# tyb311/TCCT

Hardware: AMD Instinct MI355X
Metric: OCT B-scans/sec fwd+bwd(+clip+AdamW), stc_tt bs=8 1x800x1100 (higher is better)
Workload: dtype bf16; 1 GPU; stc_tt --los=di bs=8/GPU 1x800x1100 (net tensors 3x800x1104); global_batch=8, parallelism=dp1, ranks=1, grad_allreduce=none, slowest_step=88

## Files before the change

### include/tcct_hip.h

```cpp
#ifndef TCCT_HIP_H
#define TCCT_HIP_H
#include <stdint.h>
#ifdef __cplusplus
extern "C" {
#endif

typedef void* tcct_stream_t;

enum { TCCT_F32 = 0, TCCT_BF16 = 1 };
enum { TCCT_ACT_NONE = 0, TCCT_ACT_LRELU = 1, TCCT_ACT_HSWISH = 2, TCCT_ACT_GELU = 3, TCCT_ACT_SIGMOID = 4,
       TCCT_ACT_ABS = 5 };
enum { TCCT_CRIT_DICE = 0, TCCT_CRIT_DICE2 = 1, TCCT_CRIT_IOU = 2, TCCT_CRIT_MSE = 3 };
enum { TCCT_MCRIT_DICE = 0, TCCT_MCRIT_DICE2 = 1, TCCT_MCRIT_IOU = 2, TCCT_MCRIT_CE = 3 };

int tcct_version(void);
const char* tcct_last_error(void);
int tcct_set_outputs_prezeroed(int on);

int tcct_image_to_nhwc4(const float* img, void* out, int N, int Csrc, int H, int Wsrc, int Wdst, int dtype,
                        tcct_stream_t stream);
int tcct_u8_gather2d(const uint8_t* src, uint8_t* dst, int N, int SH, int SW, int C, int sy0, int sx0, int sh, int sw, int DH, int DW,
                     int dy0, int dx0, int dh, int dw, int flipy, int flipx, int mul, int div, int fill, tcct_stream_t stream);
int tcct_onehot_to_index(const int64_t* onehot, uint8_t* lab, int N, int C, int64_t HW, tcct_stream_t stream);
int tcct_labels_to_u8(const int64_t* lab, uint8_t* out, int N, int H, int Wsrc, int Wdst, tcct_stream_t stream);
// ... 199 lines not shown
int tcct_c3_wgrad(const void* x4, const void* dy, float* dw, float* dbias, int B, int H, int W, int stride, tcct_stream_t stream);
int tcct_c3_bn_fwd_train(const void* x4, const float* w, const float* bias, void* z, int B, int H, int W, int stride, double* sums,
                         const float* gamma, const float* beta, float eps, float momentum, float* running_mean, float* running_var,
                         int64_t* num_batches_tracked, float* mean_rstd, float* ab, int post_act, tcct_stream_t stream);
int tcct_c3_bn_fwd_eval(const void* x4, const float* w, const float* bias, void* z, int B, int H, int W, int stride, const float* ab, int post_act,
                        tcct_stream_t stream);
int tcct_c3_bn_bwd_reduce(const void* x4, const float* w, const float* bias, const void* dz, int B, int H, int W, int stride, const float* ab,
                          double* raw, int post_act, tcct_stream_t stream);
int tcct_c3_bn_bwd_wgrad(const void* x4, const float* w, const float* bias, const void* dz, int B, int H, int W, int stride, const float* coef,
                         float* dw, float* dbias, int post_act, tcct_stream_t stream);
int64_t tcct_c3_bn_bwd_prefetch(int tiles_ahead);
int tcct_c3_bn_bwd_onepass(const void* x4, const float* w, const float* bias, const void* dz, int B, int H, int W, int stride, const float* mean_rstd,
                           const float* ab, float* work, double* sums, float* dw, float* dbias, float* dgamma, float* dbeta, int post_act, tcct_stream_t stream);
int tcct_pw_wgrad_smalln(const void* x, const void* dy, float* dw, float* dbias, int64_t M, int K, int N, int x_dtype,
                         int dy_dtype, tcct_stream_t stream);

int tcct_stream_copy(const void* src, void* dst, int64_t nbytes, tcct_stream_t stream);

int64_t tcct_kernel_census(int which, int reset);
int tcct_marker(int id, tcct_stream_t stream);

int tcct_dwconv3x3_fwd(const void* x, const float* w, const float* bias, void* y, int N, int H, int W, int C,
                       int stride, int add_input, int dtype, tcct_stream_t stream);
int tcct_dwconv3x3_fwd_bnstats(const void* x, const float* w, const float* bias, void* y, int N, int H, int W, int C, int stride,
                               int add_input, double* stats, int dtype, tcct_stream_t stream);
int tcct_dwconv3x3_dgrad(const void* dy, const float* w, void* dx, int N, int H, int W, int C, int stride,
                         int add_input, int dtype, tcct_stream_t stream);
int tcct_dwconv3x3_dgrad_add(const void* dy, const float* w, const void* res, void* dx, int N, int H, int W, int C, int stride,
                             int add_input, int dtype, tcct_stream_t stream);
int tcct_dwconv3x3_wgrad(const void* x, const void* dy, float* dw, float* dbias, int N, int H, int W, int C,
                         int stride, int dtype, tcct_stream_t stream);
int tcct_dwconv3x3_fwd_xaff(const void* x, const float* xab, const float* w, const float* bias, void* y, int N, int H, int W, int C, int stride,
                            double* stats, int dtype, tcct_stream_t stream);
int tcct_dwconv3x3_wgrad_xaff(const void* x, const float* xab, const void* dy, float* dw, float* dbias, int N, int H, int W, int C, int stride, int dtype,
                              tcct_stream_t stream);
int tcct_dwconv3x3_dgrad_bnred(const void* dy, const float* w, const void* y_prev, const float* ab_prev, void* dx, double* raw, int N, int H, int W, int C,
                               int dtype, tcct_stream_t stream);

int tcct_metapool_fwd(const void* x, void* y, int B, int64_t N, int C, int dtype, tcct_stream_t stream);
int tcct_metapool_bwd(const void* dy, void* dx, int B, int64_t N, int C, int dtype, tcct_stream_t stream);
int tcct_metapool_residual_fwd(const void* x, const void* res, const float* scale, void* y, int B, int64_t N, int C, int dtype,
                               tcct_stream_t stream);
int tcct_metapool_scaled_bwd(const void* dy, const float* scale, void* dx, int B, int64_t N, int C, int dtype, tcct_stream_t stream);
int tcct_ln_metapool_residual_fwd(const void* t, void* y, int B, int64_t N, int C, const float* gamma, const float* beta, float eps, const float* scale,
                                  int dtype, tcct_stream_t stream);
int tcct_ln_metapool_residual_ln_fwd(const void* t, void* y, void* y2, int B, int64_t N, int C, const float* gamma, const float* beta, float eps,
                                     const float* scale, const float* gamma2, const float* beta2, float eps2, float* mean_rstd2, int dtype, tcct_stream_t stream);
int tcct_ln_metapool_residual_bwd(const void* t, const void* dy, void* dt, int B, int64_t N, int C, const float* gamma, float eps, const float* scale,
                                  float* dgamma, float* dbeta, int dtype, tcct_stream_t stream);
int tcct_maxpool2_fwd(const void* x, void* y, int N, int H, int W, int C, int dtype, tcct_stream_t stream);
int tcct_maxpool2_bwd(const void* x, const void* dy, void* dx, int N, int H, int W, int C, int dtype, tcct_stream_t stream);
int tcct_maxpool2_bwd_add(const void* x, const void* dy, const void* res, void* dx, int N, int H, int W, int C, int dtype,
                          tcct_stream_t stream);
int tcct_bilinear_fwd(const void* x, void* y, int N, int H, int W, int C, int Ho, int Wo, int align_corners, int dtype,
                      tcct_stream_t stream);
int tcct_bilinear_bwd_separable(const float* dy, float* dx, float* workspace, int N, int H, int W, int C, int Ho, int Wo,
                                int align_corners, tcct_stream_t stream);
int tcct_bilinear_add_fwd(const void* x, const void* res, void* y, int N, int H, int W, int C, int Ho, int Wo, int align_corners,
                          int dtype, tcct_stream_t stream);
int64_t tcct_bilinear_bwd_x2(int on);
int tcct_bilinear_bwd(const void* dy, void* dx, int N, int H, int W, int C, int Ho, int Wo, int align_corners, int dtype,
                      tcct_stream_t stream);
int tcct_l2norm_fwd(const void* x, void* y, int64_t M, int C, float eps, int dtype, tcct_stream_t stream);
int tcct_l2norm_bwd(const void* x, const void* dy, void* dx, int64_t M, int C, float eps, int dtype, tcct_stream_t stream);
int tcct_l2norm_bwd_scaled(const void* x, const void* dy, void* dx, int64_t M, int C, float eps, float scale, int dtype,
                           tcct_stream_t stream);
int tcct_l2norm_bwd_scaled_add(const void* x, const void* dy, const void* res, void* dx, int64_t M, int C, float eps, float scale, int dtype,
                               tcct_stream_t stream);
int tcct_normadd_fwd(const void* g0, const void* g1, const void* g2, float* inv1, float* inv2, void* out, int N, int H, int W, int C,
                     int h1, int w1, int h2, int w2, float eps, int dtype, tcct_stream_t stream);
int tcct_normadd6_fwd(const void* a0, const void* b0, const void* a1, const void* b1, const void* a2, const void* b2, float* inv1, float* inv2,
                      void* out, int N, int H, int W, int C, int h1, int w1, int h2, int w2, float eps, int dtype, tcct_stream_t stream);
int tcct_l2norm_bwd2_scaled(const void* xa, const void* xb, const void* dn, const void* res_a, const void* res_b, void* da, void* db,
                            int64_t M, int C, float eps, float scale, int dtype, tcct_stream_t stream);

int tcct_softmax_dice_fwd(const void* logits, const uint8_t* labels, int64_t M, int C, double* sums, float* loss,
                          int dtype, tcct_stream_t stream);
int tcct_softmax_dice_bwd(const void* logits, const uint8_t* labels, int64_t M, int C, const double* sums,
                          const float* grad_out, float grad_scale, void* dlogits, int dtype, tcct_stream_t stream);
int tcct_updice_fwd(const float* low, const uint8_t* labels, int B, int h, int w, int H, int W, int C, double* sums, float* loss,
                    tcct_stream_t stream);
int tcct_updice_bwd(const float* low, const uint8_t* labels, int B, int h, int w, int H, int W, int C, const double* sums,
                    const float* grad_out, float grad_scale, float* ws, float* dlow, tcct_stream_t stream);
int tcct_dice_ds_fwd(const void* logits, int dtype, const uint8_t* labels, int B, int H, int W, int C, const float* low1, int h1, int w1, const float* low2,
                     int h2, int w2, const float* low3, int h3, int w3, float coff, double* sums, float* loss, tcct_stream_t stream);
int tcct_softmax_crit_fwd(const void* logits, const uint8_t* labels, int64_t M, int C, int kind, const float* class_w, double* sums, float* loss, int dtype,
                          tcct_stream_t stream);
int tcct_softmax_crit_bwd(const void* logits, const uint8_t* labels, int64_t M, int C, int kind, const float* class_w, const double* sums, const float* grad_out,
                          float grad_scale, void* dlogits, int dtype, tcct_stream_t stream);
int tcct_upcrit_fwd(const float* low, const uint8_t* labels, int B, int h, int w, int H, int W, int C, int kind, const float* class_w, double* sums, float* loss,
                    tcct_stream_t stream);
int tcct_upcrit_bwd(const float* low, const uint8_t* labels, int B, int h, int w, int H, int W, int C, int kind, const float* class_w, const double* sums,
                    const float* grad_out, float grad_scale, float* ws, float* dlow, tcct_stream_t stream);
int tcct_crit_ds_fwd(const void* logits, int dtype, const uint8_t* labels, int B, int H, int W, int C, const float* low1, int h1, int w1, const float* low2, int h2, int w2,
                     const float* low3, int h3, int w3, float coff, int kind, const float* class_w, double* sums, float* loss, tcct_stream_t stream);
int tcct_softmax_mcrit_fwd(const void* logits, const uint8_t* labels, int B, int64_t HW, int C, int kind, const float* class_w, double* sums, float* loss, int dtype,
                           tcct_stream_t stream);
int tcct_softmax_mcrit_bwd(const void* logits, const uint8_t* labels, int B, int64_t HW, int C, int kind, const float* class_w, const double* sums, const float* grad_out,
                           float grad_scale, void* dlogits, int dtype, tcct_stream_t stream);
int tcct_upmcrit_fwd(const float* low, const uint8_t* labels, int B, int h, int w, int H, int W, int C, int kind, const float* class_w, double* sums, float* loss,
                     tcct_stream_t stream);
int tcct_upmcrit_bwd(const float* low, const uint8_t* labels, int B, int h, int w, int H, int W, int C, int kind, const float* class_w, const double* sums,
                     const float* grad_out, float grad_scale, float* ws, float* dlow, tcct_stream_t stream);
int tcct_mcrit_ds_fwd(const void* logits, int dtype, const uint8_t* labels, int B, int H, int W, int C, const float* low1, int h1, int w1, const float* low2, int h2, int w2,
                      const float* low3, int h3, int w3, float coff, int kind, const float* class_w, double* sums, float* loss, tcct_stream_t stream);
int tcct_softmax_pick(const void* logits, const uint8_t* labels, int64_t M, int C, float* prob_lab, uint8_t* argmax,
                      int dtype, tcct_stream_t stream);
int tcct_confusion_counts(const uint8_t* pred, const uint8_t* labels, int N, int64_t HW, int C, float* out,
                          tcct_stream_t stream);

int tcct_gate_fusion_fwd(const void* x1, const void* x2, const float* field, void* y, int N, int H, int W, int C, int hs, int ws,
                         int dtype, tcct_stream_t stream);
int tcct_gate_fusion_bwd(const void* dy, const float* field, void* dx1, void* dx2, int N, int H, int W, int C, int hs, int ws,
                         int dtype, tcct_stream_t stream);

int tcct_mask_boundaries(const uint8_t* mask, int32_t* out, int N, int H, int W, int C, tcct_stream_t stream);

int tcct_eval_counts(const void* pred, int pred_kind, const uint8_t* labels, int B, int H, int W, int C, int h_valid, int w_valid, int32_t* counts, int32_t* bnd_pred,
                     int32_t* bnd_lab, uint8_t* argmax, tcct_stream_t stream);
int tcct_eval_scores(const int32_t* counts, const int32_t* bnd_pred, const int32_t* bnd_lab, int B, int C, int W, int h_valid, int w_valid, double* table,
                     tcct_stream_t stream);
int tcct_ordered_decode(const void* logits, int kind, int B, int H, int W, int C, int h_valid, int w_valid, void* take_ws, uint8_t* mask, int32_t* bnd,
                        int32_t* changed, int32_t* best, tcct_stream_t stream);
int64_t tcct_layout_decode_ws_bytes(int B, int H, int W, int S, int n_free);
int tcct_layout_decode(const void* pred, int kind, int B, int H, int W, int C, const int* layers, int S, int free_mask, int h_valid, int w_valid, void* ws,
                       uint8_t* mask, int32_t* bnd, int32_t* changed, int32_t* best, uint8_t* state, tcct_stream_t stream);
int tcct_eval_layout_scores(const int32_t* counts, const int32_t* bnd_pred, const int32_t* bnd_lab, int B, int C, int S, int W, int h_valid, int w_valid,
                            double* table, tcct_stream_t stream);
int64_t tcct_layout_marginals_ws_bytes(int B, int H, int W, int S, int n_free);
int tcct_layout_marginals(const void* logits, int kind, int B, int H, int W, int C, const int* layers, int S, int free_mask, int h_valid, int w_valid, float tau,
                          void* ws, float* surf, float* var, float* logz, float* post, tcct_stream_t stream);
int tcct_eval_soft_scores(const float* surf, const float* var, const int32_t* bnd_lab, int B, int S, int W, int h_valid, int w_valid, double* table,
                          tcct_stream_t stream);

int tcct_slice_channels_fwd(const void* x, float* y, int64_t M, int C, int start, int n, int dtype, tcct_stream_t stream);
int tcct_slice_channels_bwd(const float* dy, void* dx, int64_t M, int C, int start, int n, int dtype, tcct_stream_t stream);
int tcct_label_planes(const uint8_t* labels, float* onehot, float* edge, int N, int H, int W, int start, int n,
                      tcct_stream_t stream);
int tcct_gumbel_colsoftmax_fwd(const float* x, const float* eps, float* out, float* stats, int N, int H, int W, int CH,
                               tcct_stream_t stream);
int tcct_gumbel_colsoftmax_bwd(const float* x, const float* eps, const float* stats, const float* dout, float* dx, int N,
                               int H, int W, int CH, tcct_stream_t stream);
int tcct_colsoftmax_fwd(const float* x, float* y, int N, int H, int W, tcct_stream_t stream);
int tcct_colsoftmax_bwd(const float* y, const float* dy, float* dx, int N, int H, int W, tcct_stream_t stream);
int tcct_colwsum_fwd(const float* x, const float* wts, float* out, int N, int H, int W, tcct_stream_t stream);
int tcct_colwsum_bwd(const float* dout, const float* wts, float* dx, int N, int H, int W, tcct_stream_t stream);
int tcct_mse_fwd(const float* a, const float* b, int64_t n, double* acc, float* out, tcct_stream_t stream);
int tcct_mse_bwd(const float* a, const float* b, int64_t n, const float* grad_out, float grad_scale, float* da, float* db,
                 tcct_stream_t stream);

int64_t tcct_fpl_select_workspace_bytes();
int tcct_fpl_select(const void* feat, const uint8_t* labels, const float* prob, int64_t M, int C, void* workspace, uint32_t* counts,
                    uint8_t* binmap, float* pro_sum, int dtype, tcct_stream_t stream);
int tcct_fpl_loss(const float* pro_sum, const uint32_t* counts, const float* buf_grad, int C, float* pro, float* loss, float* dpro_over_n,
                  tcct_stream_t stream);
int tcct_fpl_backward(const uint8_t* labels, const uint8_t* binmap, const float* dpro_over_n, const float* grad_out,
                      float grad_scale, int64_t M, void* dfeat, int dtype, tcct_stream_t stream);
int tcct_l2norm_bwd_fplgrad(const void* x, const uint8_t* labels, const uint8_t* binmap, const float* dpro_over_n, const float* grad_out,
                            float grad_scale, int ncls, const void* res, void* dx, int64_t M, float eps, float scale, int dtype, tcct_stream_t stream);
int tcct_bilinear_bwd_fplgrad(const uint8_t* labels, const uint8_t* binmap, const float* dpro_over_n, const float* grad_out, float grad_scale, int ncls,
                              void* dx, int N, int H, int W, int Ho, int Wo, int align_corners, int dtype, tcct_stream_t stream);
int tcct_l2norm_bwd2_fplgrad(const void* xa, const void* xb, const uint8_t* labels, const uint8_t* binmap, const float* dpro_over_n,
                             const float* grad_out, float grad_scale, int ncls, const void* res_a, const void* res_b, void* da, void* db,
                             int64_t M, float eps, float scale, int dtype, tcct_stream_t stream);

int64_t tcct_fatt_kstats_workspace_bytes(int B, int64_t N, int C);
// ... 42 lines not shown
```

### tcct_amd/csrc/loss.hip

```cpp
#include "common.h"

#define LB 256
#define MAXC 5
#define MCNS mc5
#include "loss_classes.inc"
#undef MCNS
#undef MAXC
#define MAXC 8

#define MCNS mc8
#include "loss_classes.inc"
#undef MCNS
#undef MAXC
#define MAXC 16
#define MCNS mc16
#include "loss_classes.inc"
#undef MCNS

#define DICE_BY_C(CALL) (C == 5 ? mc5::CALL : (C <= 8 ? mc8::CALL : mc16::CALL))
#define PICK_BY_C(CALL) (C <= 8 ? mc8::CALL : mc16::CALL)

extern "C" int tcct_softmax_dice_fwd(const void* logits, const uint8_t* labels, int64_t M, int C, double* sums, float* loss, int dtype, tcct_stream_t stream) {
    return DICE_BY_C(tcct_softmax_dice_fwd_impl(logits, labels, M, C, sums, loss, dtype, stream));
}
extern "C" int tcct_softmax_dice_bwd(const void* logits, const uint8_t* labels, int64_t M, int C, const double* sums, const float* grad_out, float grad_scale, void* dlogits, int dtype, tcct_stream_t stream) {
    return DICE_BY_C(tcct_softmax_dice_bwd_impl(logits, labels, M, C, sums, grad_out, grad_scale, dlogits, dtype, stream));
}
extern "C" int tcct_updice_fwd(const float* low, const uint8_t* labels, int B, int h, int w, int H, int W, int C, double* sums, float* loss, tcct_stream_t stream) {
    return DICE_BY_C(tcct_updice_fwd_impl(low, labels, B, h, w, H, W, C, sums, loss, stream));
}
extern "C" int tcct_updice_bwd(const float* low, const uint8_t* labels, int B, int h, int w, int H, int W, int C, const double* sums, const float* grad_out, float grad_scale, float* ws, float* dlow, tcct_stream_t stream) {
    return DICE_BY_C(tcct_updice_bwd_impl(low, labels, B, h, w, H, W, C, sums, grad_out, grad_scale, ws, dlow, stream));
}
extern "C" int tcct_dice_ds_fwd(const void* logits, int dtype, const uint8_t* labels, int B, int H, int W, int C, const float* low1, int h1, int w1,
                                const float* low2, int h2, int w2, const float* low3, int h3, int w3, float coff, double* sums, float* loss,
                                tcct_stream_t stream) {
    const float* lows[3] = {low1, low2, low3};
    const int lh[3] = {h1, h2, h3}, lw[3] = {w1, w2, w3};
    const int nlow = low1 ? (low2 ? (low3 ? 3 : 2) : 1) : 0;
    return DICE_BY_C(tcct_dice_ds_fwd_impl(logits, dtype, labels, B, H, W, C, lows, lh, lw, nlow, coff, sums, loss, stream));
}
extern "C" int tcct_softmax_pick(const void* logits, const uint8_t* labels, int64_t M, int C, float* prob_lab, uint8_t* argmax, int dtype, tcct_stream_t stream) {
    return PICK_BY_C(tcct_softmax_pick_impl(logits, labels, M, C, prob_lab, argmax, dtype, stream));
}
extern "C" int tcct_confusion_counts(const uint8_t* pred, const uint8_t* labels, int N, int64_t HW, int C, float* out, tcct_stream_t stream) {
    return PICK_BY_C(tcct_confusion_counts_impl(pred, labels, N, HW, C, out, stream));
}

template <typename T>
__global__ void k_slice_fwd(const T* __restrict__ x, float* __restrict__ y, int64_t M, int C, int start, int n) {
    for (int64_t i = (int64_t)blockIdx.x * blockDim.x + threadIdx.x; i < M * n; i += (int64_t)gridDim.x * blockDim.x)
        y[i] = ldf(x + (i / n) * C + start + (i % n));
}
template <typename T>
__global__ void k_slice_bwd(const float* __restrict__ dy, T* __restrict__ dx, int64_t M, int C, int start, int n) {
    for (int64_t i = (int64_t)blockIdx.x * blockDim.x + threadIdx.x; i < M * C; i += (int64_t)gridDim.x * blockDim.x) {
        int c = (int)(i % C) - start;
        stf(dx + i, (c >= 0 && c < n) ? dy[(i / C) * n + c] : 0.f);
    }
}
extern "C" int tcct_slice_channels_fwd(const void* x, float* y, int64_t M, int C, int start, int n, int dtype, tcct_stream_t stream) {
    TCCT_CHECK(start >= 0 && n > 0 && start + n <= C, "slice_channels_fwd: bad range");
    TCCT_DISPATCH(dtype, hipLaunchKernelGGL(k_slice_fwd<T>, dim3(tcct_grid(M * n, LB, 1 << 16)), dim3(LB), 0, (hipStream_t)stream, (const T*)x, y, M, C, start, n));
    TCCT_LAUNCH_OK();
}
extern "C" int tcct_slice_channels_bwd(const float* dy, void* dx, int64_t M, int C, int start, int n, int dtype, tcct_stream_t stream) {
    TCCT_CHECK(start >= 0 && n > 0 && start + n <= C, "slice_channels_bwd: bad range");
    TCCT_DISPATCH(dtype, hipLaunchKernelGGL(k_slice_bwd<T>, dim3(tcct_grid(M * C, LB, 1 << 16)), dim3(LB), 0, (hipStream_t)stream, dy, (T*)dx, M, C, start, n));
    TCCT_LAUNCH_OK();
}

__global__ void k_label_planes(const uint8_t* __restrict__ lab, float* __restrict__ onehot, float* __restrict__ edge, int N,
                               int H, int W, int start, int n) {
    const int64_t total = (int64_t)N * H * W;
    for (int64_t i = (int64_t)blockIdx.x * blockDim.x + threadIdx.x; i < total; i += (int64_t)gridDim.x * blockDim.x) {
        int l = lab[i];
        if (onehot)
            for (int c = 0; c < n; ++c) onehot[i * n + c] = (l == start + c) ? 1.f : 0.f;
        if (edge) {
            int h = (int)((i / W) % H);
            float e = 0.f;
            if (h > 0) {
                int lp = lab[i - W];
                int cnt = 0;
                if (l != lp) { cnt += (l >= start && l < start + n); cnt += (lp >= start && lp < start + n); }
                e = cnt > 0 ? 1.f : 0.f;
            }
            edge[i] = e;
        }
    }
}
extern "C" int tcct_label_planes(const uint8_t* labels, float* onehot, float* edge, int N, int H, int W, int start, int n,
                                 tcct_stream_t stream) {
    hipLaunchKernelGGL(k_label_planes, dim3(tcct_grid((int64_t)N * H * W, LB, 1 << 16)), dim3(LB), 0, (hipStream_t)stream, labels, onehot, edge, N, H, W, start, n);
    TCCT_LAUNCH_OK();
}

#define GSEG 8
__device__ __forceinline__ float gumbel_z(float x, float e) { return x - 0.5f * logf(-logf(e)); }

template <int CH>
__global__ void __launch_bounds__(64 * GSEG)
k_gumbel_fwd(const float* __restrict__ x, const float* __restrict__ eps, float* __restrict__ out,
             float* __restrict__ stats, int N, int H, int W) {
    __shared__ float sm[GSEG][64], sz[GSEG][64];
    const int WC = W * CH;
    const int64_t cols = (int64_t)N * WC;
    const int lane = threadIdx.x & 63, seg = threadIdx.x >> 6;
    const int64_t col = (int64_t)blockIdx.x * 64 + lane;
    const bool ok = col < cols;
    const int64_t cc = ok ? col : 0;
    const int64_t n = cc / WC;
    const int wc = (int)(cc % WC);
    const float* xp = x + n * (int64_t)H * WC + wc;
    const float* ep = eps + n * (int64_t)H * WC + wc;
// ... 281 lines not shown
```

### tcct_amd/csrc/loss_classes.inc

```
namespace MCNS {
#include "loss_device.inc"
__device__ __forceinline__ void dice_accum(float (&z)[MAXC], int C, int l, float (&I)[MAXC], float (&P)[MAXC], float (&G)[MAXC]) {
    softmax_inplace(z, C);
#pragma unroll
    for (int c = 0; c < MAXC; ++c) {
        P[c] += z[c];
        if (c == l) { I[c] += z[c]; G[c] += 1.f; }
    }
}
#define DSB 1024
template <typename T>
__global__ void __launch_bounds__(DSB) k_dice_sums(const T* __restrict__ logits, const uint8_t* __restrict__ lab, int64_t M, int C,
                            double* __restrict__ sums ) {
    float I[MAXC], P[MAXC], G[MAXC];
#pragma unroll
    for (int c = 0; c < MAXC; ++c) I[c] = P[c] = G[c] = 0.f;
    for (int64_t i = (int64_t)blockIdx.x * blockDim.x + threadIdx.x; i < M; i += (int64_t)gridDim.x * blockDim.x) {
        float z[MAXC];
#pragma unroll
        for (int c = 0; c < MAXC; ++c) z[c] = c < C ? ldf(logits + i * C + c) : -INFINITY;
        dice_accum(z, C, lab[i], I, P, G);
    }
    sums_block_tail<DSB>(I, P, G, C, sums);
}
// ... 18 lines not shown
    __shared__ float s_k[2 * MAXC];
    if ((int)threadIdx.x < C) {
        const int c = threadIdx.x;
        const double U = 1.0 + sums[C + c] + sums[2 * C + c];
        s_k[c] = (float)(-2.0 / U);
        s_k[MAXC + c] = (float)((1.0 + 2.0 * sums[c]) / (U * U));
    }
    __syncthreads();
#pragma unroll
    for (int c = 0; c < MAXC; ++c) { ka[c] = c < C ? s_k[c] : 0.f; kb[c] = c < C ? s_k[MAXC + c] : 0.f; }
}

template <typename T>
__global__ void k_dice_bwd(const T* __restrict__ logits, const uint8_t* __restrict__ lab, int64_t M, int C,
                           const double* __restrict__ sums, const float* __restrict__ gout, float gscale,
                           T* __restrict__ dlogits) {
    float a[MAXC], b[MAXC];
    const float gs = gscale * (gout ? *gout : 1.f);
    dice_grad_coeffs(sums, C, a, b);
    for (int64_t i = (int64_t)blockIdx.x * blockDim.x + threadIdx.x; i < M; i += (int64_t)gridDim.x * blockDim.x) {
        float z[MAXC], mx = -INFINITY;
#pragma unroll
        for (int c = 0; c < MAXC; ++c) { z[c] = c < C ? ldf(logits + i * C + c) : -INFINITY; mx = fmaxf(mx, z[c]); }
        float s = 0.f;
#pragma unroll
        for (int c = 0; c < MAXC; ++c) { z[c] = c < C ? __expf(z[c] - mx) : 0.f; s += z[c]; }
        float inv = __builtin_amdgcn_rcpf(s);
        int l = lab[i];
        float dp[MAXC], dot = 0.f;
#pragma unroll
        for (int c = 0; c < MAXC; ++c) { z[c] *= inv; dp[c] = b[c] + (c == l ? a[c] : 0.f); dot += z[c] * dp[c]; }
#pragma unroll
        for (int c = 0; c < MAXC; ++c)
            if (c < C) stf(dlogits + i * C + c, gs * z[c] * (dp[c] - dot));
    }
}
static int tcct_softmax_dice_bwd_impl(const void* logits, const uint8_t* labels, int64_t M, int C, const double* sums,
                                     const float* grad_out, float grad_scale, void* dlogits, int dtype, tcct_stream_t stream) {
    TCCT_CHECK(C >= 2 && C <= MAXC, "softmax_dice_bwd: C=%d unsupported", C);
    TCCT_DISPATCH(dtype, hipLaunchKernelGGL(k_dice_bwd<T>, dim3(tcct_grid(M, LB, 1 << 16)), dim3(LB), 0, (hipStream_t)stream, (const T*)logits, labels, M, C, sums, grad_out, grad_scale, (T*)dlogits));
    TCCT_LAUNCH_OK();
}

template <int S>
__global__ void __launch_bounds__(UDB) k_updice_sums(const float* __restrict__ low, const uint8_t* __restrict__ lab, int B, int h, int w,
                                                     int H, int W, int C, float sh, double* __restrict__ sums) {
    float I[MAXC], P[MAXC], G[MAXC];
#pragma unroll
    for (int c = 0; c < MAXC; ++c) I[c] = P[c] = G[c] = 0.f;
    const int items = B * H * w;
    const uint32_t m_w = w > 1 ? (uint32_t)((1ull << 32) / (uint32_t)w) : 0xffffffffu, m_H = H > 1 ? (uint32_t)((1ull << 32) / (uint32_t)H) : 0xffffffffu;
    for (int base = blockIdx.x * UDB + (threadIdx.x & ~63); base < items; base += gridDim.x * UDB) {
        const bool live = base + (int)(threadIdx.x & 63) < items;
        const int it = live ? base + (int)(threadIdx.x & 63) : items - 1;
        const int row = (int)udiv32(it, w, m_w), j = it - row * w;
        const int n = (int)udiv32(row, H, m_H), ho = row - n * H;
        float R[3][MAXC];
        updice_rows<S>(low, n, h, w, C, src_index(ho, sh, h, 0), j, R, live);
        if (!live) continue;
        const uint8_t* lr = lab + (int64_t)row * W + S * j;
#pragma unroll
        for (int k = 0; k < S; ++k) {
            float z[MAXC];
            updice_pixel<S>(R, k + S / 2, C, z);
            dice_accum(z, C, lr[k], I, P, G);
        }
    }
    sums_block_tail<UDB>(I, P, G, C, sums);
}
static int dice_launch_upsums(const char* what, const float* low, const uint8_t* labels, int B, int h, int w, int H, int W, int C, double* sums, hipStream_t st) {
    int Sc;
    if (int rc = upsampled_args_ok(what, B, h, w, H, W, &Sc)) return rc;
    UPDICE_SCALES(Sc, hipLaunchKernelGGL(k_updice_sums<S>, dim3(tcct_grid((int64_t)B * H * w, UDB, 512)), dim3(UDB), 0, st, low, labels, B, h, w, H, W, C, (float)h / (float)H, sums));
    return 0;
}
static int tcct_updice_fwd_impl(const float* low, const uint8_t* labels, int B, int h, int w, int H, int W, int C, double* sums,
                               float* loss, tcct_stream_t stream) {
    TCCT_CHECK(C >= 2 && C <= MAXC, "updice_fwd: C=%d unsupported (2..%d)", C, MAXC);
    hipStream_t st = (hipStream_t)stream;
    if (hipMemsetAsync(sums, 0, sizeof(double) * 3 * C, st) != hipSuccess) { tcct_set_error("updice_fwd: memset failed"); return -2; }
    if (int rc = dice_launch_upsums("updice_fwd", low, labels, B, h, w, H, W, C, sums, st)) return rc;
    hipLaunchKernelGGL(k_dice_finalize, dim3(1), dim3(64), 0, st, sums, C, loss);
    TCCT_LAUNCH_OK();
}
template <int S>
__global__ void __launch_bounds__(256) k_updice_bwd_w(const float* __restrict__ low, const uint8_t* __restrict__ lab, int B, int h, int w,
                                                      int H, int W, int C, float sh, const double* __restrict__ sums,
                                                      const float* __restrict__ gout, float gscale, float* __restrict__ T) {
    float ka[MAXC], kb[MAXC];
    const float gs = gscale * (gout ? *gout : 1.f);
    dice_grad_coeffs(sums, C, ka, kb);
    const int lane = threadIdx.x & 63;
    const int wpr = (w + 61) / 62;
    const int nwaves = B * H * wpr;
    const uint32_t m_p = wpr > 1 ? (uint32_t)((1ull << 32) / (uint32_t)wpr) : 0xffffffffu, m_H = H > 1 ? (uint32_t)((1ull << 32) / (uint32_t)H) : 0xffffffffu;
    for (int wv = blockIdx.x * 4 + (int)(threadIdx.x >> 6); wv < nwaves; wv += gridDim.x * 4) {
        const int row = (int)udiv32(wv, wpr, m_p), wir = wv - row * wpr;
        const int n = (int)udiv32(row, H, m_H), ho = row - n * H;
        const int jj = 62 * wir - 1 + lane;
        const bool live = jj >= 0 && jj < w;
        const int j = live ? jj : (jj < 0 ? 0 : w - 1);
        const Lerp a = src_index(ho, sh, h, 0);
        float R[3][MAXC];
        updice_rows<S>(low, n, h, w, C, a, j, R, live);
        float own[MAXC], tlo[MAXC], thi[MAXC];
#pragma unroll
        for (int c = 0; c < MAXC; ++c) own[c] = tlo[c] = thi[c] = 0.f;
        if (live) {
            const uint8_t* lr = lab + (int64_t)row * W + S * j;
#pragma unroll
            for (int k = 0; k < S; ++k) {
                const float f = ((float)k + 0.5f) / (float)S;
                const bool left = k < S / 2;
                const float l1 = left ? f + 0.5f : f - 0.5f, l0 = 1.f - l1;
                float z[MAXC];
                updice_pixel<S>(R, k + S / 2, C, z);
                softmax_inplace(z, C);
                const int l = lr[k];
                float dp[MAXC], dot = 0.f;
#pragma unroll
                for (int c = 0; c < MAXC; ++c) { dp[c] = kb[c] + (c == l ? ka[c] : 0.f); dot += z[c] * dp[c]; }
                const float w_own = left ? (j == 0 ? 1.f : l1) : (j == w - 1 ? 1.f : l0);
                const float w_oth = left ? (j == 0 ? 0.f : l0) : (j == w - 1 ? 0.f : l1);
#pragma unroll
                for (int c = 0; c < MAXC; ++c) {
                    const float g = gs * z[c] * (dp[c] - dot);
                    own[c] += w_own * g;
                    if (left) tlo[c] += w_oth * g; else thi[c] += w_oth * g;
                }
            }
        }
#pragma unroll
        for (int c = 0; c < MAXC; ++c) {
            const float from_left = __shfl_up(thi[c], 1, 64), from_right = __shfl_down(tlo[c], 1, 64);
            own[c] = (from_left + own[c]) + from_right;
        }
        if (live && lane >= 1 && lane <= 62) {
            float* t = T + ((int64_t)row * w + j) * C;
#pragma unroll
            for (int c = 0; c < MAXC; ++c)
                if (c < C) t[c] = own[c];
        }
    }
}
static int tcct_updice_bwd_impl(const float* low, const uint8_t* labels, int B, int h, int w, int H, int W, int C, const double* sums,
                               const float* grad_out, float grad_scale, float* ws, float* dlow, tcct_stream_t stream) {
    TCCT_CHECK(C >= 2 && C <= MAXC, "updice_bwd: C=%d unsupported", C);
    int Sc;
    if (int rc = upsampled_args_ok("updice_bwd", B, h, w, H, W, &Sc)) return rc;
    TCCT_CHECK(ws != nullptr, "updice_bwd: workspace [B,H,w,C] fp32 is NULL");
    hipStream_t st = (hipStream_t)stream;
    UPDICE_SCALES(Sc, hipLaunchKernelGGL(k_updice_bwd_w<S>, dim3(tcct_grid((int64_t)B * H * ((w + 61) / 62), 4, 1 << 14)), dim3(256), 0, st, low, labels, B, h, w, H, W, C, (float)h / (float)H,
                                         sums, grad_out, grad_scale, ws));
    launch_updice_bwd_h(ws, B, h, w, C, H, Sc, dlow, st);
    TCCT_LAUNCH_OK();
}

template <typename T>
__global__ void k_softmax_pick(const T* __restrict__ logits, const uint8_t* __restrict__ lab, int64_t M, int C,
                               float* __restrict__ prob_lab, uint8_t* __restrict__ argmax) {
    for (int64_t i = (int64_t)blockIdx.x * blockDim.x + threadIdx.x; i < M; i += (int64_t)gridDim.x * blockDim.x) {
        float z[MAXC], mx = -INFINITY;
        int am = 0;
#pragma unroll
        for (int c = 0; c < MAXC; ++c) {
            z[c] = c < C ? ldf(logits + i * C + c) : -INFINITY;
            if (z[c] > mx) { mx = z[c]; am = c; }
        }
        if (argmax) argmax[i] = (uint8_t)am;
        if (prob_lab) {
            float s = 0.f, pl = 0.f;
            int l = lab[i];
#pragma unroll
            for (int c = 0; c < MAXC; ++c) { float e = c < C ? __expf(z[c] - mx) : 0.f; s += e; if (c == l) pl = e; }
            prob_lab[i] = pl / s;
        }
    }
}
static int tcct_softmax_pick_impl(const void* logits, const uint8_t* labels, int64_t M, int C, float* prob_lab,
                                 uint8_t* argmax, int dtype, tcct_stream_t stream) {
    TCCT_CHECK(C >= 2 && C <= MAXC, "softmax_pick: C=%d unsupported", C);
    TCCT_CHECK(!(prob_lab && !labels), "softmax_pick: prob_lab needs labels");
    TCCT_DISPATCH(dtype, hipLaunchKernelGGL(k_softmax_pick<T>, dim3(tcct_grid(M, LB, 1 << 16)), dim3(LB), 0, (hipStream_t)stream, (const T*)logits, labels, M, C, prob_lab, argmax));
    TCCT_LAUNCH_OK();
}

__global__ void k_confusion(const uint8_t* __restrict__ pred, const uint8_t* __restrict__ lab, int64_t HW, int C,
                            float* __restrict__ out ) {
    __shared__ float sm[3 * MAXC];
    const int n = blockIdx.y;
    if (threadIdx.x < 3 * MAXC) sm[threadIdx.x] = 0.f;
    __syncthreads();
    float I[MAXC], P[MAXC], G[MAXC];
#pragma unroll
    for (int c = 0; c < MAXC; ++c) I[c] = P[c] = G[c] = 0.f;
    for (int64_t i = (int64_t)blockIdx.x * blockDim.x + threadIdx.x; i < HW; i += (int64_t)gridDim.x * blockDim.x) {
        int p = pred[n * HW + i], l = lab[n * HW + i];
#pragma unroll
        for (int c = 0; c < MAXC; ++c) { P[c] += (p == c); G[c] += (l == c); I[c] += (p == c && l == c); }
    }
#pragma unroll
    for (int c = 0; c < MAXC; ++c) {
        float a = wave_sum(I[c]), b = wave_sum(P[c]), g = wave_sum(G[c]);
        if ((threadIdx.x & 63) == 0) { atomicAdd(&sm[c * 3], a); atomicAdd(&sm[c * 3 + 1], b); atomicAdd(&sm[c * 3 + 2], g); }
    }
    __syncthreads();
    if (threadIdx.x < 3 * C) atomicAdd(&out[(int64_t)n * C * 3 + threadIdx.x], sm[threadIdx.x]);
}
static int tcct_confusion_counts_impl(const uint8_t* pred, const uint8_t* labels, int N, int64_t HW, int C, float* out,
                                     tcct_stream_t stream) {
    TCCT_CHECK(C >= 1 && C <= MAXC, "confusion_counts: C=%d unsupported", C);
    hipStream_t st = (hipStream_t)stream;
    if (hipMemsetAsync(out, 0, sizeof(float) * N * C * 3, st) != hipSuccess) { tcct_set_error("confusion_counts: memset failed"); return -2; }
    dim3 grid(tcct_grid(HW, LB, 256), N);
    hipLaunchKernelGGL(k_confusion, grid, dim3(LB), 0, st, pred, labels, HW, C, out);
    TCCT_LAUNCH_OK();
}

__global__ void k_dice_finalize_ds(const double* __restrict__ sums, int C, int nheads, float coff, float* __restrict__ loss) {
    if (threadIdx.x == 0) {
        float t = 0.f;
        for (int i = nheads - 1; i >= 0; --i) {
            const double* sm = sums + (size_t)i * 3 * C;
            double l = 0.0;
            for (int c = 0; c < C; ++c) l += 1.0 - (1.0 + 2.0 * sm[c]) / (1.0 + sm[C + c] + sm[2 * C + c]);
            t = i > 0 ? t + (float)l * coff : t + (float)l;
        }
        *loss = t;
    }
}
static int tcct_dice_ds_fwd_impl(const void* logits, int dtype, const uint8_t* labels, int B, int H, int W, int C, const float* const* lows, const int* lh,
                                 const int* lw, int nlow, float coff, double* sums, float* loss, tcct_stream_t stream) {
    TCCT_CHECK(C >= 2 && C <= MAXC && nlow >= 0 && nlow <= 3, "dice_ds_fwd: C=%d (2..%d), %d low-resolution heads (0..3)", C, MAXC, nlow);
    hipStream_t st = (hipStream_t)stream;
    if (hipMemsetAsync(sums, 0, sizeof(double) * 3 * C * (1 + nlow), st) != hipSuccess) { tcct_set_error("dice_ds_fwd: memset failed"); return -2; }
    const int64_t M = (int64_t)B * H * W;
    TCCT_DISPATCH(dtype, hipLaunchKernelGGL(k_dice_sums<T>, dim3(tcct_grid(M, DSB, 512)), dim3(DSB), 0, st, (const T*)logits, labels, M, C, sums));
// ... 7 lines not shown
```

### tcct_amd/csrc/loss_device.inc

```
__device__ __forceinline__ void softmax_inplace(float (&z)[MAXC], int C) {
    float mx = -INFINITY, s = 0.f;
#pragma unroll
    for (int c = 0; c < MAXC; ++c) mx = fmaxf(mx, z[c]);
#pragma unroll
    for (int c = 0; c < MAXC; ++c) { z[c] = c < C ? __expf(z[c] - mx) : 0.f; s += z[c]; }
    const float inv = __builtin_amdgcn_rcpf(s);
#pragma unroll
    for (int c = 0; c < MAXC; ++c) z[c] *= inv;
}
struct TailPlain {
    __device__ __forceinline__ bool keep(int) const { return true; }
    __device__ __forceinline__ double scale(int, double a) const { return a; }
};
template <int NB, typename Hook = TailPlain>
__device__ __forceinline__ void sums_block_tail(const float (&A)[MAXC], const float (&P)[MAXC], const float (&G)[MAXC], int C, double* __restrict__ sums ,
                                                Hook hook = Hook()) {
    __shared__ float sm[3 * MAXC][NB / 64];
    const int w = threadIdx.x >> 6, lane = threadIdx.x & 63;
#pragma unroll
    for (int c = 0; c < MAXC; ++c) {
        float a = wave_sum(A[c]), b = wave_sum(P[c]), g = wave_sum(G[c]);
        if (lane == 0) { sm[c][w] = a; sm[MAXC + c][w] = b; sm[2 * MAXC + c][w] = g; }
    }
    __syncthreads();
    if (threadIdx.x < 3 * MAXC) {
        int q = threadIdx.x / MAXC, c = threadIdx.x % MAXC;
        if (c < C && hook.keep(q)) {
            double a = 0.0;
            for (int k = 0; k < NB / 64; ++k) a += (double)sm[threadIdx.x][k];
            atomicAdd(&sums[q * C + c], hook.scale(c, a));
        }
    }
}
#define UDB 1024
__device__ __forceinline__ uint32_t udiv32(int n, int d, uint32_t m) {
    uint32_t q = __umulhi((uint32_t)n, m);
    if ((uint32_t)n - q * (uint32_t)d >= (uint32_t)d) ++q;
    return q;
}
template <int S>
__device__ __forceinline__ void updice_rows(const float* __restrict__ low, int n, int h, int w, int C, const Lerp& a, int j, float (&R)[3][MAXC], bool live = true) {
    const float* r0 = low + ((int64_t)n * h + a.i0) * w * C;
    const float* r1 = low + ((int64_t)n * h + a.i1) * w * C;
    const int lane = threadIdx.x & 63;
#pragma unroll
    for (int c = 0; c < MAXC; ++c) R[1][c] = (live && c < C) ? a.l0 * r0[j * C + c] + a.l1 * r1[j * C + c] : -INFINITY;
    const bool nb_lo = __shfl_up((int)live, 1, 64) != 0 && lane > 0, nb_hi = __shfl_down((int)live, 1, 64) != 0 && lane < 63;
#pragma unroll
    for (int c = 0; c < MAXC; ++c) {
        const float lo = __shfl_up(R[1][c], 1, 64), hi = __shfl_down(R[1][c], 1, 64);
        R[0][c] = j == 0 ? R[1][c] : lo;
        R[2][c] = j == w - 1 ? R[1][c] : hi;
    }
    const bool miss_lo = live && j > 0 && !nb_lo, miss_hi = live && j < w - 1 && !nb_hi;
    if (miss_lo) {
#pragma unroll
        for (int c = 0; c < MAXC; ++c) R[0][c] = c < C ? a.l0 * r0[(j - 1) * C + c] + a.l1 * r1[(j - 1) * C + c] : -INFINITY;
    }
    if (miss_hi) {
#pragma unroll
        for (int c = 0; c < MAXC; ++c) R[2][c] = c < C ? a.l0 * r0[(j + 1) * C + c] + a.l1 * r1[(j + 1) * C + c] : -INFINITY;
    }
}
template <int S>
__device__ __forceinline__ void updice_pixel(const float (&R)[3][MAXC], int kk , int C, float (&z)[MAXC]) {
    const int k = (kk + S / 2) % S;
    const float f = ((float)k + 0.5f) / (float)S;
    const float l1 = k < S / 2 ? f + 0.5f : f - 0.5f, l0 = 1.f - l1;
    const int q = kk < S ? 0 : 1;
#pragma unroll
    for (int c = 0; c < MAXC; ++c) z[c] = c < C ? l0 * R[q][c] + l1 * R[q + 1][c] : -INFINITY;
}
#define UPDICE_SCALES(S_, STMT) \
    do { if (S_ == 2) { constexpr int S = 2; STMT; } else if (S_ == 4) { constexpr int S = 4; STMT; } else if (S_ == 8) { constexpr int S = 8; STMT; } \
         else { constexpr int S = 16; STMT; } } while (0)
static int upsampled_args_ok(const char* what, int B, int h, int w, int H, int W, int* Sc) {
    *Sc = h > 0 ? H / h : 0;
    TCCT_CHECK(B >= 1 && h >= 1 && w >= 1 && H == *Sc * h && W == *Sc * w && (*Sc == 2 || *Sc == 4 || *Sc == 8 || *Sc == 16),
               "%s: needs an integer scale 2/4/8/16 (got %dx%d -> %dx%d)", what, h, w, H, W);
    TCCT_CHECK((int64_t)B * H * w < (1LL << 31), "%s: tensor too large", what);
    return 0;
}
__global__ void k_updice_bwd_h(const float* __restrict__ T, int B, int h, int wC, int H, int S, float sh, float* __restrict__ dlow) {
    const int e = blockIdx.x * blockDim.x + threadIdx.x;
    if (e >= wC) return;
    for (int row = blockIdx.y; row < B * h; row += gridDim.y) {
        const int n = row / h, i = row - n * h;
        const int o0 = max(0, S * i - S / 2), o1 = min(H - 1, S * i + (3 * S) / 2 - 1);
        float acc = 0.f;
        for (int o = o0; o <= o1; ++o) {
            const Lerp a = src_index(o, sh, h, 0);
            const float wt = (a.i0 == i ? a.l0 : 0.f) + (a.i1 == i ? a.l1 : 0.f);
            acc += wt * T[((int64_t)n * H + o) * wC + e];
        }
        dlow[(int64_t)row * wC + e] = acc;
    }
}
static void launch_updice_bwd_h(const float* ws, int B, int h, int w, int C, int H, int S, float* dlow, hipStream_t st) {
    const int wC = w * C, gx2 = (wC + 255) / 256;
    int gy2 = B * h; if (gy2 > 65535) gy2 = 65535;
    hipLaunchKernelGGL(k_updice_bwd_h, dim3(gx2, gy2), dim3(256), 0, st, ws, B, h, wC, H, S, (float)h / (float)H, dlow);
}
```

Before: 431.9 B-scans/s.

## Fuse upsampled-dice backward width and height passes into a row-strip kernel

Adds a strip kernel for the upsampled dice-loss backward. Each wave walks a strip of low-res rows, recomputes the upsampled softmax gradient row by row, and accumulates the vertical interpolation weights in registers before writing dlow directly. This removes the full [B,H,w,C] fp32 workspace write and the separate height-reduction kernel, and loads labels as packed words. By default it is used for scales 2 and 4, with a mode switch to fall back to the old path. Risks include less parallelism per wave, a serial loop over output rows, and fp-contract changes that alter rounding.

```diff
diff --git a/include/tcct_hip.h b/include/tcct_hip.h
--- a/include/tcct_hip.h
+++ b/include/tcct_hip.h
@@ -305,6 +305,7 @@
                     tcct_stream_t stream);
 int tcct_updice_bwd(const float* low, const uint8_t* labels, int B, int h, int w, int H, int W, int C, const double* sums,
                     const float* grad_out, float grad_scale, float* ws, float* dlow, tcct_stream_t stream);
+int64_t tcct_updice_bwd_mode(int mode);
 int tcct_dice_ds_fwd(const void* logits, int dtype, const uint8_t* labels, int B, int H, int W, int C, const float* low1, int h1, int w1, const float* low2,
                      int h2, int w2, const float* low3, int h3, int w3, float coff, double* sums, float* loss, tcct_stream_t stream);
 int tcct_softmax_crit_fwd(const void* logits, const uint8_t* labels, int64_t M, int C, int kind, const float* class_w, double* sums, float* loss, int dtype,
diff --git a/tcct_amd/csrc/loss.hip b/tcct_amd/csrc/loss.hip
--- a/tcct_amd/csrc/loss.hip
+++ b/tcct_amd/csrc/loss.hip
@@ -1,6 +1,7 @@
 #include "common.h"
 
 #define LB 256
+static int g_updice_bwd_mode = 0;
 #define MAXC 5
 #define MCNS mc5
 #include "loss_classes.inc"
@@ -31,6 +32,11 @@
 }
 extern "C" int tcct_updice_bwd(const float* low, const uint8_t* labels, int B, int h, int w, int H, int W, int C, const double* sums, const float* grad_out, float grad_scale, float* ws, float* dlow, tcct_stream_t stream) {
     return DICE_BY_C(tcct_updice_bwd_impl(low, labels, B, h, w, H, W, C, sums, grad_out, grad_scale, ws, dlow, stream));
+}
+extern "C" int64_t tcct_updice_bwd_mode(int mode) {
+    const int prev = g_updice_bwd_mode;
+    if (mode >= 0 && mode <= 64) g_updice_bwd_mode = mode;
+    return prev;
 }
 extern "C" int tcct_dice_ds_fwd(const void* logits, int dtype, const uint8_t* labels, int B, int H, int W, int C, const float* low1, int h1, int w1,
                                 const float* low2, int h2, int w2, const float* low3, int h3, int w3, float coff, double* sums, float* loss,
diff --git a/tcct_amd/csrc/loss_classes.inc b/tcct_amd/csrc/loss_classes.inc
--- a/tcct_amd/csrc/loss_classes.inc
+++ b/tcct_amd/csrc/loss_classes.inc
@@ -124,6 +124,44 @@
     if (int rc = dice_launch_upsums("updice_fwd", low, labels, B, h, w, H, W, C, sums, st)) return rc;
     hipLaunchKernelGGL(k_dice_finalize, dim3(1), dim3(64), 0, st, sums, C, loss);
     TCCT_LAUNCH_OK();
+}
+template <int S>
+__device__ __forceinline__ void updice_bwd_item(const float (&R)[3][MAXC], const uint32_t (&lw)[(S + 3) / 4], const float (&ka)[MAXC], const float (&kb)[MAXC], float gs,
+                                                int j, int w, int C, bool live, float (&own)[MAXC]) {
+#pragma clang fp contract(off)
+    float tlo[MAXC], thi[MAXC];
+#pragma unroll
+    for (int c = 0; c < MAXC; ++c) own[c] = tlo[c] = thi[c] = 0.f;
+    if (live) {
+#pragma unroll
+        for (int k = 0; k < S; ++k) {
+            const float f = ((float)k + 0.5f) / (float)S;
+            const bool left = k < S / 2;
+            const float l1 = left ? f + 0.5f : f - 0.5f, l0 = 1.f - l1;
+            const int q = left ? 0 : 1;
+            float z[MAXC];
+#pragma unroll
+            for (int c = 0; c < MAXC; ++c) z[c] = c < C ? fmaf(l0, R[q][c], l1 * R[q + 1][c]) : -INFINITY;
+            softmax_inplace(z, C);
+            const int l = updice_label<S>(lw, k);
+            float dp[MAXC], dot = 0.f;
+#pragma unroll
+            for (int c = 0; c < MAXC; ++c) { dp[c] = kb[c] + (c == l ? ka[c] : 0.f); dot = fmaf(z[c], dp[c], dot); }
+            const float w_own = left ? (j == 0 ? 1.f : l1) : (j == w - 1 ? 1.f : l0);
+            const float w_oth = left ? (j == 0 ? 0.f : l0) : (j == w - 1 ? 0.f : l1);
+#pragma unroll
+            for (int c = 0; c < MAXC; ++c) {
+                const float g = gs * z[c] * (dp[c] - dot);
+                own[c] = fmaf(w_own, g, own[c]);
+                if (left) tlo[c] = fmaf(w_oth, g, tlo[c]); else thi[c] = fmaf(w_oth, g, thi[c]);
+            }
+        }
+    }
+#pragma unroll
+    for (int c = 0; c < MAXC; ++c) {
+        const float from_left = __shfl_up(thi[c], 1, 64), from_right = __shfl_down(tlo[c], 1, 64);
+        own[c] = (from_left + own[c]) + from_right;
+    }
 }
 template <int S>
 __global__ void __launch_bounds__(256) k_updice_bwd_w(const float* __restrict__ low, const uint8_t* __restrict__ lab, int B, int h, int w,
@@ -144,47 +182,114 @@
         const int j = live ? jj : (jj < 0 ? 0 : w - 1);
         const Lerp a = src_index(ho, sh, h, 0);
         float R[3][MAXC];
-        updice_rows<S>(low, n, h, w, C, a, j, R, live);
-        float own[MAXC], tlo[MAXC], thi[MAXC];
-#pragma unroll
-        for (int c = 0; c < MAXC; ++c) own[c] = tlo[c] = thi[c] = 0.f;
-        if (live) {
-            const uint8_t* lr = lab + (int64_t)row * W + S * j;
-#pragma unroll
-            for (int k = 0; k < S; ++k) {
-                const float f = ((float)k + 0.5f) / (float)S;
-                const bool left = k < S / 2;
-                const float l1 = left ? f + 0.5f : f - 0.5f, l0 = 1.f - l1;
-                float z[MAXC];
-                updice_pixel<S>(R, k + S / 2, C, z);
-                softmax_inplace(z, C);
-                const int l = lr[k];
-                float dp[MAXC], dot = 0.f;
-#pragma unroll
-                for (int c = 0; c < MAXC; ++c) { dp[c] = kb[c] + (c == l ? ka[c] : 0.f); dot += z[c] * dp[c]; }
-                const float w_own = left ? (j == 0 ? 1.f : l1) : (j == w - 1 ? 1.f : l0);
-                const float w_oth = left ? (j == 0 ? 0.f : l0) : (j == w - 1 ? 0.f : l1);
+        updice_rows<S, true>(low, n, h, w, C, a, j, R, live);
+        uint32_t lw[(S + 3) / 4];
+        updice_load_labels<S>(lab + (int64_t)row * W + S * j, false, lw);
+        float own[MAXC];
+        updice_bwd_item<S>(R, lw, ka, kb, gs, j, w, C, live, own);
+        if (live && lane >= 1 && lane <= 62) {
+            float* t = T + ((int64_t)row * w + j) * C;
+#pragma unroll
+            for (int c = 0; c < MAXC; ++c)
+                if (c < C) t[c] = own[c];
+        }
+    }
+}
+template <int S>
+__global__ void __launch_bounds__(256) k_updice_bwd_strip(const float* __restrict__ low, const uint8_t* __restrict__ lab, int B, int h, int w,
+                                                          int H, int W, int C, float sh, const double* __restrict__ sums,
+                                                          const float* __restrict__ gout, float gscale, int RS, int lab_al, float* __restrict__ dlow) {
+    float ka[MAXC], kb[MAXC];
+    const float gs = gscale * (gout ? *gout : 1.f);
+    dice_grad_coeffs(sums, C, ka, kb);
+    const int lane = threadIdx.x & 63;
+    const int wpr = (w + 61) / 62, nstrips = (h + RS - 1) / RS;
+    const int wv = __builtin_amdgcn_readfirstlane(blockIdx.x * 4 + (int)(threadIdx.x >> 6));
+    if (wv >= B * nstrips * wpr) return;
+    const int ns = wv / wpr, wir = wv - ns * wpr;
+    const int n = ns / nstrips, ia = (ns - n * nstrips) * RS, ib = min(h, ia + RS);
+    const int jj = 62 * wir - 1 + lane;
+    const bool live = jj >= 0 && jj < w;
+    const int j = live ? jj : (jj < 0 ? 0 : w - 1);
+    const bool nb_lo = __shfl_up((int)live, 1, 64) != 0 && lane > 0, nb_hi = __shfl_down((int)live, 1, 64) != 0 && lane < 63;
+    const bool miss_lo = live && j > 0 && !nb_lo, miss_hi = live && j < w - 1 && !nb_hi;
+    const bool miss = miss_lo || miss_hi;
+    const int jx = miss_lo ? j - 1 : (miss_hi ? j + 1 : j);
+    const int o_lo = max(0, S * ia - S / 2), o_hi = min(H - 1, S * (ib - 1) + (3 * S) / 2 - 1);
+    const float* ln = low + (int64_t)n * h * w * C;
+    const uint8_t* lr = lab + (int64_t)n * H * W + S * j;
+    Lerp a = src_index(o_lo, sh, h, 0);
+    float L0[MAXC], L1[MAXC], X0[MAXC], X1[MAXC];
+#pragma unroll
+    for (int c = 0; c < MAXC; ++c) {
+        L0[c] = c < C ? ln[((int64_t)a.i0 * w + j) * C + c] : 0.f;
+        L1[c] = c < C ? ln[((int64_t)a.i1 * w + j) * C + c] : 0.f;
+        X0[c] = (miss && c < C) ? ln[((int64_t)a.i0 * w + jx) * C + c] : 0.f;
+        X1[c] = (miss && c < C) ? ln[((int64_t)a.i1 * w + jx) * C + c] : 0.f;
+    }
+    uint32_t nl[(S + 3) / 4];
+    updice_load_labels<S>(lr + (int64_t)o_lo * W, lab_al != 0, nl);
+    float acc0[MAXC], acc1[MAXC];
+#pragma unroll
+    for (int c = 0; c < MAXC; ++c) acc0[c] = acc1[c] = 0.f;
+    for (int o = o_lo; o <= o_hi; ++o) {
+        float R[3][MAXC];
+#pragma unroll
+        for (int c = 0; c < MAXC; ++c) R[1][c] = (live && c < C) ? updice_lerp(a.l0, L0[c], a.l1, L1[c]) : -INFINITY;
+#pragma unroll
+        for (int c = 0; c < MAXC; ++c) {
+            const float lo = __shfl_up(R[1][c], 1, 64), hi = __shfl_down(R[1][c], 1, 64);
+            R[0][c] = j == 0 ? R[1][c] : lo;
+            R[2][c] = j == w - 1 ? R[1][c] : hi;
+        }
+        if (miss_lo) {
+#pragma unroll
+            for (int c = 0; c < MAXC; ++c) R[0][c] = c < C ? updice_lerp(a.l0, X0[c], a.l1, X1[c]) : -INFINITY;
+        }
+        if (miss_hi) {
+#pragma unroll
+            for (int c = 0; c < MAXC; ++c) R[2][c] = c < C ? updice_lerp(a.l0, X0[c], a.l1, X1[c]) : -INFINITY;
+        }
+        uint32_t lw[(S + 3) / 4];
+#pragma unroll
+        for (int q = 0; q < (S + 3) / 4; ++q) lw[q] = nl[q];
+        Lerp an = a;
+        bool adv = true;
+        if (o < o_hi) {
+            an = src_index(o + 1, sh, h, 0);
+            adv = an.i0 != a.i0;
+            updice_load_labels<S>(lr + (int64_t)(o + 1) * W, lab_al != 0, nl);
+            if (adv) {
 #pragma unroll
                 for (int c = 0; c < MAXC; ++c) {
-                    const float g = gs * z[c] * (dp[c] - dot);
-                    own[c] += w_own * g;
-                    if (left) tlo[c] += w_oth * g; else thi[c] += w_oth * g;
+                    L0[c] = L1[c];
+                    X0[c] = X1[c];
+                    L1[c] = c < C ? ln[((int64_t)an.i1 * w + j) * C + c] : 0.f;
+                    X1[c] = (miss && c < C) ? ln[((int64_t)an.i1 * w + jx) * C + c] : 0.f;
                 }
             }
         }
-#pragma unroll
-        for (int c = 0; c < MAXC; ++c) {
-            const float from_left = __shfl_up(thi[c], 1, 64), from_right = __shfl_down(tlo[c], 1, 64);
-            own[c] = (from_left + own[c]) + from_right;
-        }
-        if (live && lane >= 1 && lane <= 62) {
-            float* t = T + ((int64_t)row * w + j) * C;
-#pragma unroll
-            for (int c = 0; c < MAXC; ++c)
-                if (c < C) t[c] = own[c];
-        }
-    }
-}
+        float own[MAXC];
+        updice_bwd_item<S>(R, lw, ka, kb, gs, j, w, C, live, own);
+        const int r0 = a.i0, r1 = a.i0 + 1;
+        const float wt0 = (a.i0 == r0 ? a.l0 : 0.f) + (a.i1 == r0 ? a.l1 : 0.f);
+        const float wt1 = (a.i0 == r1 ? a.l0 : 0.f) + (a.i1 == r1 ? a.l1 : 0.f);
+#pragma unroll
+        for (int c = 0; c < MAXC; ++c) { acc0[c] = fmaf(wt0, own[c], acc0[c]); acc1[c] = fmaf(wt1, own[c], acc1[c]); }
+        if (adv) {
+            if (r0 >= ia && r0 < ib && live && lane >= 1 && lane <= 62) {
+                float* d = dlow + (((int64_t)n * h + r0) * w + j) * C;
+#pragma unroll
+                for (int c = 0; c < MAXC; ++c)
+                    if (c < C) d[c] = acc0[c];
+            }
+#pragma unroll
+            for (int c = 0; c < MAXC; ++c) { acc0[c] = acc1[c]; acc1[c] = 0.f; }
+        }
+        a = an;
+    }
+}
+static int updice_strip_rows(int S) { return S == 2 ? 8 : (S == 4 ? 4 : 0); }
 static int tcct_updice_bwd_impl(const float* low, const uint8_t* labels, int B, int h, int w, int H, int W, int C, const double* sums,
                                const float* grad_out, float grad_scale, float* ws, float* dlow, tcct_stream_t stream) {
     TCCT_CHECK(C >= 2 && C <= MAXC, "updice_bwd: C=%d unsupported", C);
@@ -192,9 +297,18 @@
     if (int rc = upsampled_args_ok("updice_bwd", B, h, w, H, W, &Sc)) return rc;
     TCCT_CHECK(ws != nullptr, "updice_bwd: workspace [B,H,w,C] fp32 is NULL");
     hipStream_t st = (hipStream_t)stream;
-    UPDICE_SCALES(Sc, hipLaunchKernelGGL(k_updice_bwd_w<S>, dim3(tcct_grid((int64_t)B * H * ((w + 61) / 62), 4, 1 << 14)), dim3(256), 0, st, low, labels, B, h, w, H, W, C, (float)h / (float)H,
-                                         sums, grad_out, grad_scale, ws));
-    launch_updice_bwd_h(ws, B, h, w, C, H, Sc, dlow, st);
+    const int mode = g_updice_bwd_mode;
+    const int RS = mode >= 2 ? mode : (mode == 1 ? 0 : updice_strip_rows(Sc));
+    if (RS == 0 || (MAXC >= 16 && Sc >= 8)) {
+        UPDICE_SCALES(Sc, hipLaunchKernelGGL(k_updice_bwd_w<S>, dim3(tcct_grid((int64_t)B * H * ((w + 61) / 62), 4, 1 << 14)), dim3(256), 0, st, low, labels, B, h, w, H, W, C, (float)h / (float)H,
+                                             sums, grad_out, grad_scale, ws));
+        launch_updice_bwd_h(ws, B, h, w, C, H, Sc, dlow, st);
+        TCCT_LAUNCH_OK();
+    }
+    const int64_t nwaves = (int64_t)B * ((h + RS - 1) / RS) * ((w + 61) / 62);
+    const int lab_al = ((uintptr_t)labels & (uintptr_t)(Sc - 1)) == 0;
+    UPDICE_SCALES(Sc, if constexpr (MAXC < 16 || S < 8) hipLaunchKernelGGL(k_updice_bwd_strip<S>, dim3((unsigned)((nwaves + 3) / 4)), dim3(256), 0, st, low, labels, B, h, w, H, W, C,
+                                                                           (float)h / (float)H, sums, grad_out, grad_scale, RS, lab_al, dlow));
     TCCT_LAUNCH_OK();
 }
 
diff --git a/tcct_amd/csrc/loss_device.inc b/tcct_amd/csrc/loss_device.inc
--- a/tcct_amd/csrc/loss_device.inc
+++ b/tcct_amd/csrc/loss_device.inc
@@ -38,11 +38,35 @@
     if ((uint32_t)n - q * (uint32_t)d >= (uint32_t)d) ++q;
     return q;
 }
-template <int S>
+__device__ __forceinline__ float updice_lerp(float l0, float x0, float l1, float x1) {
+#pragma clang fp contract(off)
+    return fmaf(l0, x0, l1 * x1);
+}
+template <int S, bool EXACT = false>
 __device__ __forceinline__ void updice_rows(const float* __restrict__ low, int n, int h, int w, int C, const Lerp& a, int j, float (&R)[3][MAXC], bool live = true) {
     const float* r0 = low + ((int64_t)n * h + a.i0) * w * C;
     const float* r1 = low + ((int64_t)n * h + a.i1) * w * C;
     const int lane = threadIdx.x & 63;
+    if constexpr (EXACT) {
+#pragma unroll
+        for (int c = 0; c < MAXC; ++c) R[1][c] = (live && c < C) ? updice_lerp(a.l0, r0[j * C + c], a.l1, r1[j * C + c]) : -INFINITY;
+        const bool nb_lo = __shfl_up((int)live, 1, 64) != 0 && lane > 0, nb_hi = __shfl_down((int)live, 1, 64) != 0 && lane < 63;
+#pragma unroll
+        for (int c = 0; c < MAXC; ++c) {
+            const float lo = __shfl_up(R[1][c], 1, 64), hi = __shfl_down(R[1][c], 1, 64);
+            R[0][c] = j == 0 ? R[1][c] : lo;
+            R[2][c] = j == w - 1 ? R[1][c] : hi;
+        }
+        if (live && j > 0 && !nb_lo) {
+#pragma unroll
+            for (int c = 0; c < MAXC; ++c) R[0][c] = c < C ? updice_lerp(a.l0, r0[(j - 1) * C + c], a.l1, r1[(j - 1) * C + c]) : -INFINITY;
+        }
+        if (live && j < w - 1 && !nb_hi) {
+#pragma unroll
+            for (int c = 0; c < MAXC; ++c) R[2][c] = c < C ? updice_lerp(a.l0, r0[(j + 1) * C + c], a.l1, r1[(j + 1) * C + c]) : -INFINITY;
+        }
+        return;
+    }
 #pragma unroll
     for (int c = 0; c < MAXC; ++c) R[1][c] = (live && c < C) ? a.l0 * r0[j * C + c] + a.l1 * r1[j * C + c] : -INFINITY;
     const bool nb_lo = __shfl_up((int)live, 1, 64) != 0 && lane > 0, nb_hi = __shfl_down((int)live, 1, 64) != 0 && lane < 63;
@@ -71,6 +95,22 @@
 #pragma unroll
     for (int c = 0; c < MAXC; ++c) z[c] = c < C ? l0 * R[q][c] + l1 * R[q + 1][c] : -INFINITY;
 }
+template <int S>
+__device__ __forceinline__ void updice_load_labels(const uint8_t* __restrict__ p, bool al, uint32_t (&v)[(S + 3) / 4]) {
+    if (al) {
+        if constexpr (S == 2) v[0] = *reinterpret_cast<const uint16_t*>(p);
+        else if constexpr (S == 4) v[0] = *reinterpret_cast<const uint32_t*>(p);
+        else if constexpr (S == 8) { const uint2 t = *reinterpret_cast<const uint2*>(p); v[0] = t.x; v[1] = t.y; }
+        else { const uint4 t = *reinterpret_cast<const uint4*>(p); v[0] = t.x; v[1] = t.y; v[2] = t.z; v[3] = t.w; }
+    } else {
+#pragma unroll
+        for (int q = 0; q < (S + 3) / 4; ++q) v[q] = 0u;
+#pragma unroll
+        for (int k = 0; k < S; ++k) v[k >> 2] |= (uint32_t)p[k] << (8 * (k & 3));
+    }
+}
+template <int S>
+__device__ __forceinline__ int updice_label(const uint32_t (&v)[(S + 3) / 4], int k) { return (int)((v[k >> 2] >> (8 * (k & 3))) & 0xffu); }
 #define UPDICE_SCALES(S_, STMT) \
     do { if (S_ == 2) { constexpr int S = 2; STMT; } else if (S_ == 4) { constexpr int S = 4; STMT; } else if (S_ == 8) { constexpr int S = 8; STMT; } \
          else { constexpr int S = 16; STMT; } } while (0)
```

After: 434.0 B-scans/s, median of 6. About the same (+0.5%).
